# sandyz1000/deep-insight-face

Measured on AMD Instinct MI355X. Metric: faces/sec embedding+match (112x112, 512-d), higher is better.
Workload: dtype f32; 1 GPU; configs[3]: IResNet-100 embed, batch=512/GPU (4096 on 8 GPUs), 1M gallery row-sharded; arch=iresnet100, head=v2, batch_per_gpu=512, global_batch=512, gallery_rows=1000000, gallery_rows_per_gpu=1000000, emd=512, metric=cosine, parallelism=dp1 + gallery row-shard

## Files before the change

deep-insight-face_amd/csrc/conv.hip:

```cpp
#include "gemm_core.hpp"
#include <string>
#include "dif_internal.hpp"
#include "ops.hpp"

#include <stdlib.h>

#include <atomic>
#include <mutex>
#include <set>
#include <type_traits>
#include <utility>

namespace dif {

template <int N>
__device__ __forceinline__ void wait_vmcnt() {
  static_assert(N >= 0 && N < 64, "vmcnt is a 6-bit counter");
  asm volatile("s_waitcnt vmcnt(%0)" ::"n"(N) : "memory");
}


template <int N, int RP, bool PRE, int KMODE = 0>
struct ConvALoader {
  __amdgpu_buffer_rsrc_t rsrc;
// ... 1915 lines not shown
    g_last_kernel = names.insert(std::string("conv_skp_kernel<64x64,") + am_form(AMP + 10) + ",S=" + std::to_string(S) + ">+reduce").first->c_str();
  }
  return 0;
}

template <class T>
static int launch_conv(const ConvArgs& a, hipStream_t st) {
  if constexpr (T::BM == 64 && T::BN == 64) {
    if (const int nw = mt_plan(a)) return launch_conv_mt(a, nw, st);
    if (const int S = sk2_plan(a)) {
      const int emax = (!(a.off & CONV_OFF_BD) && a.w_frag && !(a.dbg & 16384)) ? patch_applies(a) : 0;
      if (emax == PATCH_EMAX_S) return launch_conv_skp<3>(a, S, st);
      if (emax == PATCH_EMAX_L) return launch_conv_skp<5>(a, S, st);
      const bool pw1 = a.KH == 1 && a.KW == 1 && a.pad_t == 0 && a.pad_l == 0 && a.Cin % BK == 0;
      if (pw1) return a.pre_scale ? launch_conv_sk<true, 1>(a, S, st) : launch_conv_sk<false, 1>(a, S, st);
      return a.pre_scale ? launch_conv_sk<true, 0>(a, S, st) : launch_conv_sk<false, 0>(a, S, st);
    }
  }
  constexpr bool kDefaultTile = (T::BM == 64 && T::BN == 64);
  const bool pw = a.KH == 1 && a.KW == 1 && a.pad_t == 0 && a.pad_l == 0 && a.Cin % BK == 0;
  if constexpr (kDefaultTile) {
    const int64_t tiles = ((a.M + T::BM - 1) / T::BM) * (int64_t)((a.Cout + T::BN - 1) / T::BN);
    int64_t slots = 4 * (int64_t)num_cus();
    if (slots > a.sk_max_blocks) slots = a.sk_max_blocks;
    const bool bd = !(a.off & CONV_OFF_BD) && a.w_frag != nullptr;
    if (patch2d_applies(a)) {
      if (t2_applies(a)) return launch_conv_t2(a, st);
      if (bd && conv_bdp_ok(a)) return launch_conv_bdp<T, 6>(a, st);
      return bd ? launch_conv_pre<T, false, 16>(a, st) : launch_conv_pre<T, false, 6>(a, st);
    }
    if (bd && !pw) {
      int emax_tn = patch_applies(a);
      if (emax_tn == 0 && patch_shape(a) && patch_entry_bound(a, 64) <= PATCH_EMAX_X && !(a.dbg & 8192)) emax_tn = PATCH_EMAX_X;
      if (tn_applies(a, emax_tn) && (conv_bdp_ok(a) || (a.dbg & 512)))
        return emax_tn == PATCH_EMAX_X ? launch_conv_tn<PATCH_EMAX_X>(a, st)
                                       : (emax_tn == PATCH_EMAX_L ? launch_conv_tn<PATCH_EMAX_L>(a, st) : launch_conv_tn<PATCH_EMAX_S>(a, st));
    }
    if (bd && !pw && conv_bdp_ok(a)) {
      const int emax = patch_applies(a);
      if (emax == PATCH_EMAX_S) return launch_conv_bdp<T, 3>(a, st);
      if (emax == PATCH_EMAX_L) return launch_conv_bdp<T, 5>(a, st);
    }
    if (a.Cin % 4 == 0 && pipe_applies(a, tiles, a.Kpad / BK, slots)) {
      if (pw && a.pre_scale) return launch_conv_pipe<T, true, 1, 4>(a, st);
      if (pw) return launch_conv_pipe<T, false, 1, 4>(a, st);
      if (!a.pre_scale) return launch_conv_pipe<T, false, 0, 1>(a, st);
    }
  }
  if (pw && a.pre_scale) return launch_conv_pre<T, true, 1>(a, st);
  if (pw) return launch_conv_pre<T, false, 1>(a, st);
  if constexpr (kDefaultTile) {
    {
      const bool bd2 = !(a.off & CONV_OFF_BD) && a.w_frag != nullptr;
      const int emax = patch_applies(a);
      if (bd2 && conv_bdp_ok(a)) {
        if (emax == PATCH_EMAX_S) return launch_conv_bdp<T, 3>(a, st);
        if (emax == PATCH_EMAX_L) return launch_conv_bdp<T, 5>(a, st);
        if (patch2d_applies(a)) return launch_conv_bdp<T, 6>(a, st);
      }
      if (emax == PATCH_EMAX_S) return bd2 ? launch_conv_pre<T, false, 13>(a, st) : launch_conv_pre<T, false, 3>(a, st);
      if (emax == PATCH_EMAX_L) return bd2 ? launch_conv_pre<T, false, 15>(a, st) : launch_conv_pre<T, false, 5>(a, st);
      if (patch2d_applies(a)) return bd2 ? launch_conv_pre<T, false, 16>(a, st) : launch_conv_pre<T, false, 6>(a, st);
    }
  }
  if (a.pre_scale) return launch_conv_pre<T, true, 0>(a, st);
  return launch_conv_pre<T, false, 0>(a, st);
}

template <class T, bool PRE, int AM, int BF3, int LEAN>
static int launch_conv_pre_impl(const ConvArgs& a, hipStream_t st);

template <class T, bool PRE, int AM, int BF3>
static int launch_conv_pre(const ConvArgs& a, hipStream_t st) {
  const bool lean = !(a.dbg & 1024) && a.y_H == a.Ho && a.y_W == a.Wo && a.y_oy == 0 && a.y_ox == 0 && a.y_ld == a.Cout &&
                    a.y_coff == 0 && !a.y_sub && a.Cout % 4 == 0 &&
                    (!a.res || (a.res_stride == 1 && a.res_H == a.Ho && a.res_W == a.Wo)) && (int64_t)a.M * a.Cout * 4 < 0xFFFFFFF0LL;
  if constexpr (BF3) return a.y_sub ? launch_conv_pre_impl<T, PRE, AM, BF3, 2>(a, st) : launch_conv_pre_impl<T, PRE, AM, BF3, 1>(a, st);
  else return lean ? launch_conv_pre_impl<T, PRE, AM, BF3, 1>(a, st) : launch_conv_pre_impl<T, PRE, AM, BF3, 0>(a, st);
}

template <class T, bool PRE, int AM, int BF3, int LEAN>
static int launch_conv_pre_impl(const ConvArgs& a, hipStream_t st) {
  void (*kern)(const ConvArgs) = conv_igemm_kernel<T, PRE, AM, BF3, LEAN>;
  if constexpr (BF3 != 0) {
    if (a.bf_terms == 2) kern = conv_igemm_bf2_kernel<T, PRE, AM, BF3, LEAN>;
  }
  constexpr int AMP = AM % 10;
  constexpr int emax = AMP == 3 ? PATCH_EMAX_S : (AMP == 5 ? PATCH_EMAX_L : 100);
  constexpr int epi_bytes = T::BM * (T::BN + 4) * 4;
  constexpr int bd_bytes = emax * 128 > epi_bytes ? emax * 128 : epi_bytes;
  constexpr int b3p_bytes = bf3p_lds_b(T::BM) > epi_bytes ? bf3p_lds_b(T::BM) : epi_bytes;
  constexpr int lds_bytes = BF3 ? b3p_bytes
                                : (AM >= 10 ? bd_bytes : ((AMP == 3 || AMP == 5 || AMP == 6) ? patch_lds_bytes(emax) : T::LDS_BYTES));
  if (allow_dynamic_lds(reinterpret_cast<const void*>(kern), lds_bytes)) return -1;
  const int64_t tiles = ((a.M + T::BM - 1) / T::BM) * (int64_t)((a.Cout + T::BN - 1) / T::BN);
  const int KS = (BF3 && AM >= 10) ? a.Kpad / (BK * 9) : a.Kpad / BK;
  const int64_t I = tiles * KS;
  if (I >= 0x7fffffffLL) return set_error("conv: iteration space too large");
  int64_t slots = (BF3 ? 512 / T::NT : T::BLOCKS_PER_CU) * (int64_t)num_cus();
  if (slots > a.sk_max_blocks) slots = a.sk_max_blocks;
  int64_t P;
  if (tiles >= 8 * slots || a.Kpad / BK < SK_MIN_KS || (((BF3 && a.bf_terms == 2) || (a.dbg & 2048)) && tiles >= slots) || (a.dbg & 4096)) {
    P = tiles;
  } else {
    P = slots;
    if (P > (I + 3) / 4) P = (I + 3) / 4;
  }
  if (P < 1) P = 1;
  ConvArgs b = a;
  b.fd_howo = make_fastdiv(a.Ho * a.Wo);
  b.fd_wo = make_fastdiv(a.Wo);
  b.fd_cin = make_fastdiv(a.Cin);
  b.fd_kw = make_fastdiv(a.KW);
  b.fd_ks = make_fastdiv(KS);
  b.fd_taps = make_fastdiv(a.KH * a.KW);
  b.fd_wp = make_fastdiv(a.W + 2);
  b.fd_rpi = make_fastdiv(a.H + 1);
  b.fd_t2_w = make_fastdiv(a.W / 8 > 0 ? a.W / 8 : 1);
  b.fd_t2_img = make_fastdiv((a.H / 8) * (a.W / 8) > 0 ? (a.H / 8) * (a.W / 8) : 1);
  if (a.k_order == 1 && a.Cin % BK != 0) return set_error("conv: channel-block-major K order needs Cin %% 32 == 0");
  b.fd_tiles_n = make_fastdiv((a.Cout + T::BN - 1) / T::BN);
  b.epi_fast = LEAN != 0;
  hipLaunchKernelGGL(kern, dim3((unsigned)P), dim3(T::NT), lds_bytes, st, b);
  DIF_HIP(hipGetLastError());
  static const std::string label = kernel_label<T>(BF3 ? "conv_igemm_kernel[split-bf16]" : "conv_igemm_kernel", AM, PRE ? ",preact" : "");
  g_last_kernel = label.c_str();
  return 0;
}

#include "conv_winograd.hpp"

int conv_run(const ConvArgs& a, hipStream_t st) {
  if (a.M <= 0) return 0;
  if (a.Cin % 4 != 0) return set_error("conv: Cin must be a multiple of 4 (got %d)", a.Cin);
  if (a.Cout % 4 != 0) {
    if (a.res) return set_error("conv: a shortcut needs Cout %% 4 == 0 (got %d)", a.Cout);
  } else if (a.y_ld % 4 != 0 || a.y_coff % 4 != 0) {
    return set_error("conv: output view must be 16-byte aligned");
  }
  if (a.y_ld < a.y_coff + a.Cout || a.y_H < a.Ho + a.y_oy || a.y_W < a.Wo + a.y_ox)
    return set_error("conv: output view does not fit its parent tensor");
  if (a.y_sub && (a.Cout % 4 != 0 || a.y_ld != a.Cout || a.y_H != a.Ho || a.y_W != a.Wo))
    return set_error("conv: a subsampled first output needs a plain output geometry");
  if (a.Kpad % BK != 0) return set_error("conv: Kpad must be a multiple of %d", BK);
  if (a.H >= 0x3f00 || a.W >= 0x3f00) return set_error("conv: spatial size too large");
  if ((a.pre_scale == nullptr) != (a.pre_shift == nullptr)) return set_error("conv: pre_scale and pre_shift go together");
  if (!a.sk_slab || !a.sk_flag || a.sk_max_blocks < 1) return set_error("conv: stream-K workspace missing");
  {
    const int64_t howo = (int64_t)a.Ho * a.Wo;
    const int64_t span = (256 + howo - 1) / howo + 1;
    if (span * a.H * a.W * a.Cin * 4 >= 0x7fffffffLL)
      return set_error("conv: a 256-pixel tile spans more than 2 GiB of input (%dx%dx%d)", a.H, a.W, a.Cin);
  }
  if (const int wk = wino_applies(a)) return wk == 2 ? launch_conv_winow(a, st) : launch_conv_wino(a, st);
  const int form = bf3p_applies(a) * 2 + (a.Cout <= 64 ? 1 : 0);
  if (form == 2 && (a.bf_terms == 2 || (a.dbg & 128))) return launch_conv_pre<Tile<4, 1, 1, 4>, false, 13, 1>(a, st);
  switch (form) {
    case 2: return launch_conv_pre<Tile<2, 2, 2, 2>, false, 13, 1>(a, st);
    case 3: return launch_conv_pre<Tile<2, 1, 2, 2>, false, 13, 1>(a, st);
    case 4: return launch_conv_pre<Tile<2, 2, 2, 2>, false, 16, 1>(a, st);
    case 5: return launch_conv_pre<Tile<2, 1, 2, 2>, false, 16, 1>(a, st);
    default: break;
  }
  if (a.Cout <= 32 && !(a.dbg & 8388608)) return launch_conv<Tile<1, 1, 4, 1>>(a, st);
  return launch_conv<Tile<1, 1>>(a, st);
}

}
```

deep-insight-face_amd/csrc/conv_winograd.hpp:

```cpp
namespace wino {
constexpr int BN = 64;
constexpr int KC = 16;
constexpr int64_t MIN_TILES = 64 * 49;
constexpr int WIDE_MAX_HW = 112;
constexpr int64_t WIDE_MIN_IMAGES = 128;
}

template <int TT_, int CPW_, int MIN_BLOCKS_, bool EARLY_REQ_>
struct WinoW {
  static constexpr int TT = TT_;
  static constexpr int CPW = CPW_;
  static constexpr int MIN_BLOCKS = MIN_BLOCKS_;
  static constexpr bool EARLY_REQ = EARLY_REQ_;
  static constexpr int MF = TT / 32;
  static constexpr int NT = 16 / CPW * 64;
  static constexpr int STAGE = 16 * TT * wino::KC;
  static constexpr int LDS_BYTES = 2 * STAGE * 4;
  static_assert(NT / 8 == TT && CPW % 2 == 0, "one loader thread per (tile, channel pair)");
};

__device__ __forceinline__ void wino_bt4(float x0, float x1, float x2, float x3, float& o0, float& o1, float& o2, float& o3) {
  o0 = x0 - x2;
  o1 = x1 + x2;
  o2 = x2 - x1;
  o3 = x1 - x3;
}

__device__ __forceinline__ void wino_input_transform(const float (&d)[16], float (&v)[16]) {
  float t[16];
#pragma unroll
  for (int c = 0; c < 4; ++c) wino_bt4(d[c], d[4 + c], d[8 + c], d[12 + c], t[c], t[4 + c], t[8 + c], t[12 + c]);
#pragma unroll
  for (int r = 0; r < 4; ++r) wino_bt4(t[4 * r], t[4 * r + 1], t[4 * r + 2], t[4 * r + 3], v[4 * r], v[4 * r + 1], v[4 * r + 2], v[4 * r + 3]);
}

template <bool TRACE>
__device__ __forceinline__ unsigned long long wino_stamp() {
  if constexpr (TRACE) return __builtin_amdgcn_s_memrealtime();
  return 0ull;
}
__device__ __forceinline__ void wino_trace_write(const ConvArgs& a, unsigned long long c0, const unsigned long long (&ts)[5]) {
  unsigned long long* t = a.trace + (size_t)blockIdx.x * 8;
  t[0] = ts[2] - ts[1];
  t[1] = ts[1] - ts[0];
  t[2] = ts[3] - ts[2];
  t[3] = ts[4] - ts[3];
  t[4] = (unsigned long long)__builtin_amdgcn_s_getreg((31 << 11) | 4) | ((unsigned long long)__builtin_amdgcn_s_getreg((31 << 11) | 20) << 32);
  t[5] = ts[0];
  t[6] = ts[4];
  t[7] = 3 | ((__builtin_amdgcn_s_memtime() - c0) << 8);
}

template <class S, bool TRACE>
__global__ __launch_bounds__(S::NT, S::MIN_BLOCKS) void conv_wino_kernel(const ConvArgs a, int blocks_m, int nblocks) {
  constexpr int TT = S::TT, CPW = S::CPW, MF = S::MF, KC = wino::KC;
  extern __shared__ __attribute__((aligned(16))) float wino_smem[];
  const int b = xcd_remap((int)blockIdx.x, nblocks);
  const int nt = b / blocks_m, mt = b - nt * blocks_m;
  const int tid = threadIdx.x, lane = tid & 63, wave = tid >> 6;
  const int tw = a.W >> 1, tpi = (a.H >> 1) * tw, ntiles = a.N * tpi;
  const int KS = a.Cin / KC;
  unsigned long long ts[5];
  ts[0] = wino_stamp<TRACE>();
  const unsigned long long tr_c0 = TRACE ? __builtin_amdgcn_s_memtime() : 0ull;

  const int ltile = tid >> 3, cp = tid & 7;
  const int g = mt * TT + ltile;
  const bool tile_ok = g < ntiles;
  int pix0 = 0;
  unsigned vmask = 0;
  if (tile_ok) {
    const int img = g / tpi, rem = g - img * tpi, ty = rem / tw, tx = rem - ty * tw;
    pix0 = (img * a.H + 2 * ty) * a.W + 2 * tx;
#pragma unroll
    for (int p = 0; p < 16; ++p) {
      const int iy = 2 * ty - 1 + (p >> 2), ix = 2 * tx - 1 + (p & 3);
      if (iy >= 0 && iy < a.H && ix >= 0 && ix < a.W) vmask |= 1u << p;
    }
  }
  const int row_b = a.W * a.Cin * 4, pix_b = a.Cin * 4;
  const int lbase = (pix0 - a.W - 1) * pix_b + cp * 8;
  const __amdgpu_buffer_rsrc_t xrs = make_rsrc(a.x, (uint32_t)a.N * (uint32_t)(a.H * a.W) * (uint32_t)pix_b);
  auto dload = [&](int ks, f32x2 (&d)[16]) {
#pragma unroll
    for (int p = 0; p < 16; ++p) {
      const uint32_t off = ((vmask >> p) & 1u) ? (uint32_t)(lbase + (p >> 2) * row_b + (p & 3) * pix_b + ks * (KC * 4)) : OOB;
      d[p] = __builtin_bit_cast(f32x2, __builtin_amdgcn_raw_buffer_load_b64(xrs, off, 0, 0));
    }
  };
  const int vdst = ltile * KC + (((cp >> 1) ^ ((ltile >> 2) & 3)) << 2) + (cp & 1) * 2;
  auto vstore = [&](float* buf, const f32x2 (&d)[16]) {
    float d0[16], d1[16], v0[16], v1[16];
#pragma unroll
    for (int p = 0; p < 16; ++p) {
      d0[p] = d[p][0];
      d1[p] = d[p][1];
    }
    wino_input_transform(d0, v0);
    wino_input_transform(d1, v1);
#pragma unroll
    for (int c = 0; c < 16; ++c) *reinterpret_cast<f32x2*>(buf + c * (TT * KC) + vdst) = f32x2{v0[c], v1[c]};
  };

  const int h = lane >> 5, r32 = lane & 31, sw = (r32 >> 2) & 3;
  const int tiles_n = a.Cout / wino::BN;
  const __amdgpu_buffer_rsrc_t wrs = make_rsrc(a.w_wino, a.w_wino_bytes);
  const uint32_t boff0 = (uint32_t)((CPW * wave * tiles_n + nt) * KS) * 4096u + (uint32_t)lane * 16u;
  const uint32_t bstep = (uint32_t)(tiles_n * KS) * 4096u;
  f32x4 bw[2][2][2];
  auto bload = [&](int j, int ks) {
#pragma unroll
    for (int nf = 0; nf < 2; ++nf)
#pragma unroll
      for (int q = 0; q < 2; ++q)
        bw[j & 1][nf][q] = buf_load4(wrs, boff0 + (uint32_t)j * bstep + (uint32_t)ks * 4096u + (uint32_t)(nf * 2 + q) * 1024u);
  };
  int aoff[2];
#pragma unroll
  for (int q = 0; q < 2; ++q) aoff[q] = r32 * KC + (((2 * h + q) ^ sw) << 2);
  f32x4 av[2][MF][2];
  auto aread = [&](const float* buf, int j) {
#pragma unroll
    for (int mf = 0; mf < MF; ++mf)
#pragma unroll
      for (int q = 0; q < 2; ++q)
        av[j & 1][mf][q] = *reinterpret_cast<const f32x4*>(buf + (CPW * wave + j) * (TT * KC) + mf * 32 * KC + aoff[q]);
  };
  f32x16 acc[CPW][MF][2];
#pragma unroll
  for (int j = 0; j < CPW; ++j)
#pragma unroll
    for (int mf = 0; mf < MF; ++mf)
#pragma unroll
      for (int nf = 0; nf < 2; ++nf)
#pragma unroll
        for (int r = 0; r < 16; ++r) acc[j][mf][nf][r] = 0.f;
  auto mfma = [&](int j) {
#pragma unroll
    for (int q = 0; q < 2; ++q)
#pragma unroll
      for (int t = 0; t < 4; ++t)
#pragma unroll
        for (int mf = 0; mf < MF; ++mf)
#pragma unroll
          for (int nf = 0; nf < 2; ++nf)
            acc[j][mf][nf] = __builtin_amdgcn_mfma_f32_32x32x2f32(av[j & 1][mf][q][t], bw[j & 1][nf][q][t], acc[j][mf][nf], 0, 0, 0);
  };

  {
    f32x2 d[16];
    dload(0, d);
    bload(0, 0);
    bload(1, 0);
    vstore(wino_smem, d);
    lds_barrier();
    ts[1] = wino_stamp<TRACE>();
    for (int ks = 0; ks < KS; ++ks) {
      const float* cur = wino_smem + (ks & 1) * S::STAGE;
      float* nxt = wino_smem + ((ks + 1) & 1) * S::STAGE;
      const bool more = ks + 1 < KS;
      if (more) dload(ks + 1, d);
      aread(cur, 0);
      aread(cur, 1);
#pragma unroll
      for (int j = 0; j < CPW; ++j) {
        mfma(j);
        if (j + 2 < CPW) {
          aread(cur, j + 2);
          bload(j + 2, ks);
        } else if (more) {
          bload(j + 2 - CPW, ks + 1);
        }
      }
      if (more) vstore(nxt, d);
      lds_barrier();
    }
  }
  ts[2] = wino_stamp<TRACE>();

  const int c4 = cp * 4;
  const uint32_t bytes = (uint32_t)a.M * (uint32_t)a.Cout * 4u;
  const __amdgpu_buffer_rsrc_t y_rsrc = make_rsrc(a.y, a.y ? bytes : 0u);
  const __amdgpu_buffer_rsrc_t y2_rsrc = make_rsrc(a.y2, a.y2 ? bytes : 0u);
  const __amdgpu_buffer_rsrc_t res_rsrc = make_rsrc(a.res, a.res ? bytes : 0u);
  const bool has_res = a.res != nullptr;
  const int act = a.act, act2 = a.act2;
#pragma unroll
  for (int nf = 0; nf < 2; ++nf) {
    const int c = nt * wino::BN + nf * 32 + c4;
    f32x4 sc, sh, al, sc2, sh2, al2, rv[4];
    uint32_t voff[4];
    if constexpr (S::EARLY_REQ) {
      sc = load4_or(a.scale, c, 1.f), sh = load4_or(a.shift, c, 0.f), al = load4_or(a.alpha, c, 0.f);
      sc2 = load4_or(a.scale2, c, 1.f), sh2 = load4_or(a.shift2, c, 0.f), al2 = load4_or(a.alpha2, c, 0.f);
#pragma unroll
      for (int p = 0; p < 4; ++p) {
        const int pix = pix0 + (p >> 1) * a.W + (p & 1);
        voff[p] = tile_ok ? ((uint32_t)pix * (uint32_t)a.Cout + (uint32_t)c) * 4u : OOB;
        rv[p] = has_res ? buf_load4(res_rsrc, voff[p]) : f32x4{0.f, 0.f, 0.f, 0.f};
      }
      __builtin_amdgcn_sched_barrier(0);
    }
#pragma unroll
    for (int j = 0; j < CPW; ++j)
#pragma unroll
      for (int mf = 0; mf < MF; ++mf)
#pragma unroll
        for (int r = 0; r < 16; ++r)
          wino_smem[(CPW * wave + j) * (TT * 32) + (mf * 32 + frag_row(lane, r)) * 32 + r32] = acc[j][mf][nf][r];
    lds_barrier();
    f32x4 m[16];
#pragma unroll
    for (int k = 0; k < 16; ++k) m[k] = *reinterpret_cast<const f32x4*>(wino_smem + k * (TT * 32) + ltile * 32 + c4);
    f32x4 yv[4];
    {
      f32x4 s0[4], s1[4];
#pragma unroll
      for (int jj = 0; jj < 4; ++jj) {
        s0[jj] = m[jj] + m[4 + jj] + m[8 + jj];
        s1[jj] = m[4 + jj] - m[8 + jj] - m[12 + jj];
      }
      yv[0] = s0[0] + s0[1] + s0[2];
      yv[1] = s0[1] - s0[2] - s0[3];
      yv[2] = s1[0] + s1[1] + s1[2];
      yv[3] = s1[1] - s1[2] - s1[3];
    }
    if constexpr (!S::EARLY_REQ) {
      sc = load4_or(a.scale, c, 1.f), sh = load4_or(a.shift, c, 0.f), al = load4_or(a.alpha, c, 0.f);
      sc2 = load4_or(a.scale2, c, 1.f), sh2 = load4_or(a.shift2, c, 0.f), al2 = load4_or(a.alpha2, c, 0.f);
#pragma unroll
      for (int p = 0; p < 4; ++p) {
        const int pix = pix0 + (p >> 1) * a.W + (p & 1);
        voff[p] = tile_ok ? ((uint32_t)pix * (uint32_t)a.Cout + (uint32_t)c) * 4u : OOB;
        rv[p] = has_res ? buf_load4(res_rsrc, voff[p]) : f32x4{0.f, 0.f, 0.f, 0.f};
      }
    }
#pragma unroll
    for (int p = 0; p < 4; ++p) {
      f32x4 v, v2;
      epilogue4(yv[p], sc, sh, al, act, has_res, rv[p], sc2, sh2, al2, act2, v, v2);
      __builtin_amdgcn_raw_buffer_store_b128(__builtin_bit_cast(u32x4, v), y_rsrc, voff[p], 0, 0);
      __builtin_amdgcn_raw_buffer_store_b128(__builtin_bit_cast(u32x4, v2), y2_rsrc, voff[p], 0, 0);
    }
    lds_barrier();
    ts[3 + nf] = wino_stamp<TRACE>();
  }
  if constexpr (TRACE)
    if (tid == 0) wino_trace_write(a, tr_c0, ts);
}

static int wino_applies(const ConvArgs& a) {
  if (!a.w_wino || a.wino_level < 1 || a.KH != 3 || a.KW != 3 || a.stride != 1 || a.pad_t != 1 || a.pad_l != 1) return 0;
  if (a.Ho != a.H || a.Wo != a.W || (a.H & 1) || (a.W & 1)) return 0;
  const bool wide = a.H > 16 || a.W > 16;
  if (wide && (a.wino_level < 2 || a.H > wino::WIDE_MAX_HW || a.W > wino::WIDE_MAX_HW)) return 0;
  if (a.Cin % 32 != 0 || a.Cout % wino::BN != 0 || a.pre_scale || a.y_sub) return 0;
  if (!(a.y_H == a.Ho && a.y_W == a.Wo && a.y_oy == 0 && a.y_ox == 0 && a.y_ld == a.Cout && a.y_coff == 0)) return 0;
  if (a.res && (a.res_stride != 1 || a.res_H != a.Ho || a.res_W != a.Wo)) return 0;
  if ((int64_t)a.M * a.Cout * 4 >= 0x7fffffffLL || (int64_t)a.M * a.Cin * 4 >= 0x7fffffffLL) return 0;
  if ((int64_t)16 * a.Cin * a.Cout * 4 > (int64_t)a.w_wino_bytes) return 0;
  const int64_t tpi = (int64_t)(a.H / 2) * (a.W / 2);
  if (wide) return a.N * tpi >= wino::WIDE_MIN_IMAGES * tpi ? 2 : 0;
  return a.N * tpi >= wino::MIN_TILES ? 1 : 0;
}

template <class S>
static int launch_wino(const ConvArgs& a, hipStream_t st, const char* name) {
  const auto kern = a.trace ? conv_wino_kernel<S, true> : conv_wino_kernel<S, false>;
  if (allow_dynamic_lds(reinterpret_cast<const void*>(kern), S::LDS_BYTES)) return -1;
  const int64_t ntiles = (int64_t)a.N * (a.H / 2) * (a.W / 2);
  const int blocks_m = (int)((ntiles + S::TT - 1) / S::TT), tiles_n = a.Cout / wino::BN;
  const int64_t nblocks = (int64_t)blocks_m * tiles_n;
  if (nblocks >= 0x7fffffffLL) return set_error("conv: too many tiles");
  hipLaunchKernelGGL(kern, dim3((unsigned)nblocks), dim3(S::NT), S::LDS_BYTES, st, a, blocks_m, (int)nblocks);
  DIF_HIP(hipGetLastError());
  g_last_kernel = name;
  return 0;
}

static int launch_conv_wino(const ConvArgs& a, hipStream_t st) {
  if (a.wino_level >= 2 && !(a.dbg & 16777216)) return launch_wino<WinoW<32, 4, 2, true>>(a, st, "conv_wino_kernel<F(2x2,3x3),32 tiles x 64>");
  return launch_wino<WinoW<64, 2, 1, false>>(a, st, "conv_wino_kernel<F(2x2,3x3),64 tiles x 64>");
}

static int launch_conv_winow(const ConvArgs& a, hipStream_t st) {
  if (a.dbg & 65536) return launch_wino<WinoW<64, 2, 2, true>>(a, st, "conv_winow_kernel<F(2x2,3x3),64 tiles x 64>");
  return launch_wino<WinoW<32, 4, 2, true>>(a, st, "conv_winow_kernel<F(2x2,3x3),32 tiles x 64>");
}
```

deep-insight-face_amd/csrc/net.hip:

```cpp
#include "net.hpp"

#include <math.h>
#include <stdio.h>
#include <stdlib.h>
#include <string.h>

#include <algorithm>
#include <map>

#include "../../include/dif.h"
#include "dif_internal.hpp"
#include "gemm_core.hpp"

namespace dif {

static const float EPS_RESNET = 1.001e-5f;
static const float EPS_KERAS = 1e-3f;
static const float EPS_IRESNET = 1e-5f;

Net::~Net() { release_device(); }

void Net::release_device() {
  for (Lane& L : lanes) {
    if (L.stream) (void)hipStreamDestroy(L.stream);
// ... 832 lines not shown
    for (const char* const* t = option_names(); *t; ++t) known |= !strcmp(*t, key);
    if (!known) return set_error("dif_net_set_option: unknown option '%s'", key);
  }
  auto flag = [&](unsigned bit) {
    conv_off = value ? (conv_off & ~bit) : (conv_off | bit);
    return 0;
  };
  const bool pre = !finalized;
  if (!strcmp(key, "pipe")) return use_pipe = value != 0, 0;
  if (!strcmp(key, "bdp")) {
    if (value < 0 || value > 2) return set_error("dif_net_set_option: 'bdp' takes 0, 1 or 2");
    return use_bdp = value, 0;
  }
  if (!strcmp(key, "stem")) return use_stem = value != 0, 0;
  if (!strcmp(key, "dbg")) return conv_dbg = value, 0;
  if (!strcmp(key, "wino")) {
    if (value < 0 || value > 2) return set_error("dif_net_set_option: 'wino' takes 0, 1 or 2");
    return use_wino = value, 0;
  }
  if (!strcmp(key, "patch")) return flag(CONV_OFF_PATCH);
  if (!strcmp(key, "patch2d")) return flag(CONV_OFF_PATCH2D);
  if (!strcmp(key, "bd")) return flag(CONV_OFF_BD);
  if (!strcmp(key, "t2")) return flag(CONV_OFF_T2);
  if (!strcmp(key, "tn")) return flag(CONV_OFF_TN);
  if (!strcmp(key, "sk2")) return flag(CONV_OFF_SK2);
  if (!strcmp(key, "mt")) return flag(CONV_OFF_MT);
  if (!strcmp(key, "bf16x3")) {
    if (!pre && compute_bf16x3 != (value != 0))
      return set_error("dif_net_set_option: 'bf16x3' must be chosen before dif_net_finalize");
    return compute_bf16x3 = value != 0, 0;
  }
  if (!strcmp(key, "bf_terms")) {
    if (value != 2 && value != 3) return set_error("dif_net_set_option: 'bf_terms' takes 2 or 3");
    return bf_terms = value, 0;
  }
  if (!strcmp(key, "lane_prio")) {
    if (!pre) return set_error("dif_net_set_option: 'lane_prio' must be chosen before dif_net_finalize");
    return opt_lane_prio = value, 0;
  }
  if (!strcmp(key, "ysub") || !strcmp(key, "lane_split")) {
    if (!pre) return set_error("dif_net_set_option: '%s' must be chosen before dif_net_finalize", key);
    if (key[0] == 'y') use_ysub = value != 0;
    else opt_lane_split = value < 0 ? -1 : (value != 0);
    return 0;
  }
  return set_error("dif_net_set_option: option '%s' is listed but not handled", key);
}

int Net::finalize(int mb) {
  if (mb <= 0) return set_error("max_batch must be positive");
  if (const char* env = getenv("DIF_OPTIONS")) {
    std::string all(env);
    size_t pos = 0;
    while (pos < all.size()) {
      size_t end = all.find(',', pos);
      if (end == std::string::npos) end = all.size();
      const std::string kv = all.substr(pos, end - pos);
      const size_t eq = kv.find('=');
      if (eq == std::string::npos || eq == 0) return set_error("DIF_OPTIONS: expected key=value, got '%s'", kv.c_str());
      if (set_option(kv.substr(0, eq).c_str(), atoi(kv.c_str() + eq + 1))) return -1;
      pos = end + 1;
    }
  }
  for (const Param& p : params)
    if (!p.set) return set_error("parameter '%s' was never set", p.name.c_str());
  release_device();
  max_batch = mb;

  for (Op& op : ops) {
    std::vector<float> scale, shift;
    if (op.kind == OP_CONV) {
      const int taps = op.KH * op.KW;
      const int K = taps * op.Cin;
      op.Kpad = (K + BK - 1) / BK * BK;
      op.k_order = (taps > 1 && op.Cin % BK == 0 && op.Cin_true == op.Cin) ? 1 : 0;
      std::vector<float> packed((size_t)op.Cout * op.Kpad, 0.f);
      const float* w = params[op.w].data.data();
      for (int t = 0; t < taps; ++t)
        for (int ci = 0; ci < op.Cin_true; ++ci) {
          const int64_t src_row = op.chw_flatten ? ((int64_t)ci * taps + t) : ((int64_t)t * op.Cin_true + ci);
          const float* src = w + src_row * op.Cout;
          const size_t kk = op.k_order == 1 ? ((size_t)(ci / BK) * taps + t) * BK + ci % BK : (size_t)t * op.Cin + ci;
          for (int co = 0; co < op.Cout; ++co) packed[(size_t)co * op.Kpad + kk] = src[co];
        }
      if (upload(this, packed, &op.d_w)) return -1;
      op.d_w_raw = nullptr;
      op.stem_mfma = false;
      const bool stem_shape = use_stem && op.Cin_true == 3 && op.Cin == 4 && op.res < 0 && !op.pre_bn.valid() &&
                              !op.chw_flatten && tensors[op.y >= 0 ? op.y : op.y2].parent < 0;
      if (stem_shape && op.KH == 3 && op.KW == 3 && op.stride == 1 && op.pad_t == 1 && op.pad_l == 1 && op.Cout == 32) {
        if (upload(this, params[op.w].data, &op.d_w_raw)) return -1;
      } else if (stem_shape && stem_mfma_applies(op.KH, op.KW, op.stride, op.pad_t, op.pad_l, op.Cout)) {
        if (upload(this, params[op.w].data, &op.d_w_raw)) return -1;
        op.stem_mfma = true;
      }
      op.d_w3f = nullptr;
      op.w3f_bytes = 0;
      if (compute_bf16x3 && op.k_order == 1 && op.KH == 3 && op.KW == 3 && op.stride == 1 && op.pad_t == 1 && op.pad_l == 1 &&
          !op.pre_bn.valid() && conv_bf3p_form(tensors[op.x].H, tensors[op.x].W, true, op.Cout) != 0) {
        const int KS = op.Kpad / BK, NT32 = (op.Cout + 31) / 32;
        std::vector<uint16_t> wf((size_t)NT32 * KS * 3072, 0);
        size_t o = 0;
        for (int nt = 0; nt < NT32; ++nt)
          for (int ks = 0; ks < KS; ++ks)
            for (int s2 = 0; s2 < 2; ++s2) {
              uint16_t* blk = wf.data() + o;
              o += 3 * 512;
              for (int ln = 0; ln < 64; ++ln)
                for (int t = 0; t < 8; ++t) {
                  const int row = nt * 32 + (ln & 31);
                  float r = row < op.Cout ? packed[(size_t)row * op.Kpad + (size_t)ks * BK + 16 * s2 + 8 * (ln >> 5) + t] : 0.f;
                  for (int p3 = 0; p3 < 3; ++p3) {
                    const uint16_t b = f32_to_bf16_rne(r);
                    blk[p3 * 512 + ln * 8 + t] = b;
                    r -= bf16_to_f32(b);
                  }
                }
            }
        if ((uint64_t)wf.size() * 2 < 0xFFFFFFF0ull) {
          void* d = nullptr;
          DIF_HIP(hipMalloc(&d, wf.size() * sizeof(uint16_t)));
          allocs.push_back(d);
          DIF_HIP(hipMemcpy(d, wf.data(), wf.size() * sizeof(uint16_t), hipMemcpyHostToDevice));
          op.d_w3f = d;
          op.w3f_bytes = (uint32_t)(wf.size() * sizeof(uint16_t));
        }
      }
      op.d_w_frag = nullptr;
      op.w_frag_bytes = 0;
      if (!op.d_w3f && op.k_order == 1 && op.KH == 3 && op.KW == 3 && op.stride == 1 && op.pad_t == 1 && op.pad_l == 1 &&
          !op.pre_bn.valid()) {
        const int KS = op.Kpad / BK, NT32 = (op.Cout + 31) / 32;
        std::vector<float> frag((size_t)NT32 * 32 * op.Kpad, 0.f);
        size_t o = 0;
        for (int nt = 0; nt < NT32; ++nt)
          for (int ks = 0; ks < KS; ++ks)
            for (int s2 = 0; s2 < 2; ++s2)
              for (int u = 0; u < 2; ++u)
                for (int hh = 0; hh < 2; ++hh)
                  for (int nn = 0; nn < 32; ++nn)
                    for (int t = 0; t < 4; ++t, ++o) {
                      const int row = nt * 32 + nn;
                      if (row < op.Cout) frag[o] = packed[(size_t)row * op.Kpad + (size_t)ks * BK + 16 * s2 + 8 * hh + 4 * u + t];
                    }
        if ((uint64_t)frag.size() * 4 < 0xFFFFFFF0ull) {
          if (upload(this, frag, &op.d_w_frag)) return -1;
          op.w_frag_bytes = (uint32_t)(frag.size() * 4);
        }
      }
      op.d_w_wino = nullptr;
      op.w_wino_bytes = 0;
      {
        const TensorDesc& xd = tensors[op.x];
        const TensorDesc& yd = tensors[op.y >= 0 ? op.y : op.y2];
        if (use_wino && !compute_bf16x3 && op.KH == 3 && op.KW == 3 && op.stride == 1 && op.pad_t == 1 && op.pad_l == 1 &&
            !op.pre_bn.valid() && !op.chw_flatten && !op.y_sub && op.Cin_true == op.Cin && op.Cin % BK == 0 &&
            op.Cout % 64 == 0 && xd.H % 2 == 0 && xd.W % 2 == 0 && yd.H == xd.H && yd.W == xd.W &&
            ((xd.H <= 16 && xd.W <= 16) || (use_wino >= 2 && xd.H <= 112 && xd.W <= 112)) &&
            (uint64_t)16 * op.Cin * op.Cout * 4 < 0xFFFFFFF0ull) {
          static const double G[4][3] = {{1, 0, 0}, {0.5, 0.5, 0.5}, {0.5, -0.5, 0.5}, {0, 0, 1}};
          const int KS16 = op.Cin / 16, NTn = op.Cout / 64;
          std::vector<float> u((size_t)16 * op.Cin * op.Cout);
          const float* w = params[op.w].data.data();
          for (int ci = 0; ci < op.Cin; ++ci)
            for (int co = 0; co < op.Cout; ++co) {
              double gk[3][3], tg[4][3];
              for (int t = 0; t < 9; ++t) gk[t / 3][t % 3] = w[((size_t)t * op.Cin + ci) * op.Cout + co];
              for (int i = 0; i < 4; ++i)
                for (int k = 0; k < 3; ++k) tg[i][k] = G[i][0] * gk[0][k] + G[i][1] * gk[1][k] + G[i][2] * gk[2][k];
              const int ks = ci / 16, rem = ci % 16, ln = (rem / 8) * 32 + co % 32, q = (rem % 8) / 4, t4 = rem % 4;
              const int nt = co / 64, nf = (co % 64) / 32;
              for (int i = 0; i < 4; ++i)
                for (int j = 0; j < 4; ++j) {
                  const double v = tg[i][0] * G[j][0] + tg[i][1] * G[j][1] + tg[i][2] * G[j][2];
                  const size_t c = (size_t)(4 * i + j);
                  u[(((((c * NTn + nt) * KS16 + ks) * 2 + nf) * 2 + q) * 64 + ln) * 4 + t4] = (float)v;
                }
            }
          if (upload(this, u, &op.d_w_wino)) return -1;
          op.w_wino_bytes = (uint32_t)(u.size() * 4);
        }
      }
      op.d_w_f16 = nullptr;
      op.w_f16_bytes = 0;
      {
        const bool pw1 = op.KH == 1 && op.KW == 1 && op.pad_t == 0 && op.pad_l == 0 && op.Cin % BK == 0;
        if ((pw1 || (op.k_order == 1 && op.Cin % BK == 0)) && !op.d_w_raw) {
          const int nch = op.Kpad / 16, NT16 = (op.Cout + 15) / 16;
          std::vector<float> f16((size_t)NT16 * nch * 256, 0.f);
          size_t o = 0;
          for (int ct = 0; ct < NT16; ++ct)
            for (int c = 0; c < nch; ++c)
              for (int ln = 0; ln < 64; ++ln)
                for (int t = 0; t < 4; ++t, ++o) {
                  const int row = ct * 16 + (ln & 15);
                  if (row < op.Cout) f16[o] = packed[(size_t)row * op.Kpad + (size_t)c * 16 + 4 * (ln >> 4) + t];
                }
          if ((uint64_t)f16.size() * 4 < 0xFFFFFFF0ull) {
            if (upload(this, f16, &op.d_w_f16)) return -1;
            op.w_f16_bytes = (uint32_t)(f16.size() * 4);
          }
        }
      }
      fold(this, op.bn, op.bias, op.Cout, &scale, &shift);
      if (!scale.empty() && upload(this, scale, &op.d_scale)) return -1;
      if (!shift.empty() && upload(this, shift, &op.d_shift)) return -1;
      if (op.alpha >= 0 && upload(this, params[op.alpha].data, &op.d_alpha)) return -1;
      if (op.alpha < 0 && op.const_alpha != 0.f &&
          upload(this, std::vector<float>((size_t)op.Cout, op.const_alpha), &op.d_alpha))
        return -1;
    } else if (op.kind == OP_GDCTAIL) {
      if (upload(this, params[op.w].data, &op.d_w)) return -1;
      if (upload(this, params[op.w_pw].data, &op.d_w_pw)) return -1;
      if (upload(this, params[op.w_dense].data, &op.d_w_dense)) return -1;
      fold(this, op.bn, -1, op.Cin, &scale, &shift);
      if (!scale.empty() && upload(this, scale, &op.d_scale)) return -1;
      if (!shift.empty() && upload(this, shift, &op.d_shift)) return -1;
    } else if (op.kind == OP_DWFULL || op.kind == OP_DWCONV) {
      if (upload(this, params[op.w].data, &op.d_w)) return -1;
      fold(this, op.bn, -1, op.Cout, &scale, &shift);
      if (!scale.empty() && upload(this, scale, &op.d_scale)) return -1;
      if (!shift.empty() && upload(this, shift, &op.d_shift)) return -1;
    }
    if (op.pre_bn.valid()) {
      fold(this, op.pre_bn, -1, op.Cin, &scale, &shift);
      if (upload(this, scale, &op.d_pre_scale)) return -1;
      if (upload(this, shift, &op.d_pre_shift)) return -1;
    }
    if (op.y2 >= 0) {
      fold(this, op.bn2, -1, op.Cout, &scale, &shift);
      if (!scale.empty() && upload(this, scale, &op.d_scale2)) return -1;
      if (!shift.empty() && upload(this, shift, &op.d_shift2)) return -1;
      if (op.alpha2 >= 0 && upload(this, params[op.alpha2].data, &op.d_alpha2)) return -1;
    }
  }

  for (Op& P : ops) {
    if (!use_ysub || P.kind != OP_CONV || P.y < 0 || P.y2 < 0 || P.y_sub || is_output(P.y) || tensors[P.y].parent >= 0 ||
        tensors[P.y2].parent >= 0 || P.Cout % 4 != 0)
      continue;
    bool viewed = false;
    for (const TensorDesc& t : tensors) viewed |= t.parent == P.y;
    Op* reader = nullptr;
    int readers = 0;
    for (Op& D : ops) {
      if (&D == &P) continue;
      const int uses = (D.x == P.y) + (D.res == P.y) + (D.y == P.y) + (D.y2 == P.y);
      if (uses) {
        readers += uses;
        reader = &D;
      }
    }
    if (viewed || readers != 1 || reader->kind != OP_CONV || reader->x != P.y) continue;
    if (reader->KH != 1 || reader->KW != 1 || reader->stride != 2 || reader->pad_t != 0 || reader->pad_l != 0) continue;
    TensorDesc& t = tensors[P.y];
    P.y_sub = true;
    t.H = (t.H + 1) / 2;
    t.W = (t.W + 1) / 2;
    reader->stride = 1;
  }

  for (TensorDesc& t : tensors) t.first_def = t.last_use = t.buf = -1;
  auto R = [&](int t) { return t < 0 ? t : root_of(t); };
  for (int i = 0; i < (int)ops.size(); ++i) {
    const Op& op = ops[i];
    for (int t : {R(op.y), R(op.y2)})
      if (t >= 0 && tensors[t].first_def < 0) tensors[t].first_def = i;
    for (int t : {R(op.x), R(op.res), R(op.y), R(op.y2)})
      if (t >= 0) tensors[t].last_use = std::max(tensors[t].last_use, i);
  }
  tensors[output_tensor].last_use = (int)ops.size();
  for (int e : extra_outputs) tensors[e].last_use = (int)ops.size();
  buf_elems.clear();
  std::vector<int> free_list;
  for (int i = 0; i < (int)ops.size(); ++i) {
    const Op& op = ops[i];
    for (int t : {R(op.y), R(op.y2)}) {
      if (t < 0 || is_output(t) || tensors[t].buf >= 0) continue;
      const int64_t need = tensors[t].elems();
      int best = -1;
      for (int k = 0; k < (int)free_list.size(); ++k) {
        const int b = free_list[k];
        if (buf_elems[b] >= need && (best < 0 || buf_elems[b] < buf_elems[free_list[best]])) best = k;
      }
      if (best >= 0) {
        tensors[t].buf = free_list[best];
        free_list.erase(free_list.begin() + best);
      } else {
        buf_elems.push_back(need);
        tensors[t].buf = (int)buf_elems.size() - 1;
      }
    }
    for (int t : {R(op.x), R(op.res), R(op.y), R(op.y2)})
      if (t >= 0 && !is_output(t) && tensors[t].last_use == i && tensors[t].buf >= 0) {
        if (std::find(free_list.begin(), free_list.end(), tensors[t].buf) == free_list.end())
          free_list.push_back(tensors[t].buf);
      }
  }
  sk_max_blocks = conv_max_blocks();
  if (const char* e = getenv("DIF_SK_SPIN_LIMIT")) sk_spin_limit = atoi(e);
  int n_conv = 0;
  for (const Op& op : ops) n_conv += op.kind == OP_CONV;
  const double per_launch = flops_per_image() * (max_batch / 2) / (n_conv > 0 ? n_conv : 1);
  const bool long_launches = per_launch >= 10e9;
  int nl = getenv("DIF_STREAMS") ? atoi(getenv("DIF_STREAMS")) : 2;
  lane_split = (opt_lane_split >= 0 ? opt_lane_split : (long_launches ? 0 : 1)) != 0;
  if (nl < 1) nl = 1;
  if (nl > 8) nl = 8;
  if (max_batch < lane_min_images()) nl = 1;
  lanes.assign(nl, Lane());
  DIF_HIP(hipEventCreateWithFlags(&ev_start, hipEventDisableTiming));
// ... 507 lines not shown
```

Measured before the change: 8286 faces/s.

## Extend Winograd 3x3 conv to odd-sized maps and subsampled-output convs

Widens Winograd F(2x2,3x3) coverage to two shapes that previously fell back to the implicit-GEMM path. The first is odd spatial maps up to 16x16 (e.g. 7x7 in IResNet), handled by padding tiles and masking out-of-range outputs via the input validity mask. The second is convs whose first output is stride-2 subsampled (y_sub), handled by storing only the top-left pixel of each 2x2 tile. This cuts the multiply count for those layers, at the cost of wasted work on padded tiles for odd maps and a new kernel variant to validate.

After: 8560 faces/s, median of 6. 1.03x the previous value.

```diff
diff --git a/deep-insight-face_amd/csrc/conv.hip b/deep-insight-face_amd/csrc/conv.hip
--- a/deep-insight-face_amd/csrc/conv.hip
+++ b/deep-insight-face_amd/csrc/conv.hip
@@ -2091,7 +2091,8 @@
     if (span * a.H * a.W * a.Cin * 4 >= 0x7fffffffLL)
       return set_error("conv: a 256-pixel tile spans more than 2 GiB of input (%dx%dx%d)", a.H, a.W, a.Cin);
   }
-  if (const int wk = wino_applies(a)) return wk == 2 ? launch_conv_winow(a, st) : launch_conv_wino(a, st);
+  if (const int wk = wino_applies(a); wk && !(wk == 3 && (a.dbg & 33554432)))
+    return wk == 3 ? launch_conv_winox(a, st) : wk == 2 ? launch_conv_winow(a, st) : launch_conv_wino(a, st);
   const int form = bf3p_applies(a) * 2 + (a.Cout <= 64 ? 1 : 0);
   if (form == 2 && (a.bf_terms == 2 || (a.dbg & 128))) return launch_conv_pre<Tile<4, 1, 1, 4>, false, 13, 1>(a, st);
   switch (form) {
diff --git a/deep-insight-face_amd/csrc/conv_winograd.hpp b/deep-insight-face_amd/csrc/conv_winograd.hpp
--- a/deep-insight-face_amd/csrc/conv_winograd.hpp
+++ b/deep-insight-face_amd/csrc/conv_winograd.hpp
@@ -4,6 +4,8 @@
 constexpr int64_t MIN_TILES = 64 * 49;
 constexpr int WIDE_MAX_HW = 112;
 constexpr int64_t WIDE_MIN_IMAGES = 128;
+constexpr int ODD_MAX_HW = 16;
+constexpr int64_t ODD_MIN_TILES = 128 * 16;
 }
 
 template <int TT_, int CPW_, int MIN_BLOCKS_, bool EARLY_REQ_>
@@ -12,11 +14,20 @@
   static constexpr int CPW = CPW_;
   static constexpr int MIN_BLOCKS = MIN_BLOCKS_;
   static constexpr bool EARLY_REQ = EARLY_REQ_;
+  static constexpr bool ODD = false;
+  static constexpr bool YSUB = false;
   static constexpr int MF = TT / 32;
   static constexpr int NT = 16 / CPW * 64;
   static constexpr int STAGE = 16 * TT * wino::KC;
   static constexpr int LDS_BYTES = 2 * STAGE * 4;
   static_assert(NT / 8 == TT && CPW % 2 == 0, "one loader thread per (tile, channel pair)");
+};
+
+template <bool ODD_, bool YSUB_>
+struct WinoX : WinoW<32, 4, 2, true> {
+  static constexpr bool ODD = ODD_;
+  static constexpr bool YSUB = YSUB_;
+  static_assert(!(ODD_ && YSUB_), "y_sub is admitted on even maps only");
 };
 
 __device__ __forceinline__ void wino_bt4(float x0, float x1, float x2, float x3, float& o0, float& o1, float& o2, float& o3) {
@@ -57,8 +68,9 @@
   extern __shared__ __attribute__((aligned(16))) float wino_smem[];
   const int b = xcd_remap((int)blockIdx.x, nblocks);
   const int nt = b / blocks_m, mt = b - nt * blocks_m;
-  const int tid = threadIdx.x, lane = tid & 63, wave = tid >> 6;
-  const int tw = a.W >> 1, tpi = (a.H >> 1) * tw, ntiles = a.N * tpi;
+  const int tid = threadIdx.x, lane = tid & 63;
+  const int wave = (S::ODD || S::YSUB) ? __builtin_amdgcn_readfirstlane(tid >> 6) : tid >> 6;
+  const int tw = S::ODD ? (a.W + 1) >> 1 : a.W >> 1, tpi = (S::ODD ? (a.H + 1) >> 1 : a.H >> 1) * tw, ntiles = a.N * tpi;
   const int KS = a.Cin / KC;
   unsigned long long ts[5];
   ts[0] = wino_stamp<TRACE>();
@@ -180,7 +192,7 @@
 
   const int c4 = cp * 4;
   const uint32_t bytes = (uint32_t)a.M * (uint32_t)a.Cout * 4u;
-  const __amdgpu_buffer_rsrc_t y_rsrc = make_rsrc(a.y, a.y ? bytes : 0u);
+  const __amdgpu_buffer_rsrc_t y_rsrc = make_rsrc(a.y, a.y ? (S::YSUB ? (uint32_t)ntiles * (uint32_t)a.Cout * 4u : bytes) : 0u);
   const __amdgpu_buffer_rsrc_t y2_rsrc = make_rsrc(a.y2, a.y2 ? bytes : 0u);
   const __amdgpu_buffer_rsrc_t res_rsrc = make_rsrc(a.res, a.res ? bytes : 0u);
   const bool has_res = a.res != nullptr;
@@ -196,7 +208,10 @@
 #pragma unroll
       for (int p = 0; p < 4; ++p) {
         const int pix = pix0 + (p >> 1) * a.W + (p & 1);
-        voff[p] = tile_ok ? ((uint32_t)pix * (uint32_t)a.Cout + (uint32_t)c) * 4u : OOB;
+        if constexpr (S::ODD)
+          voff[p] = ((vmask >> (5 + 4 * (p >> 1) + (p & 1))) & 1u) ? ((uint32_t)pix * (uint32_t)a.Cout + (uint32_t)c) * 4u : OOB;
+        else
+          voff[p] = tile_ok ? ((uint32_t)pix * (uint32_t)a.Cout + (uint32_t)c) * 4u : OOB;
         rv[p] = has_res ? buf_load4(res_rsrc, voff[p]) : f32x4{0.f, 0.f, 0.f, 0.f};
       }
       __builtin_amdgcn_sched_barrier(0);
@@ -231,7 +246,10 @@
 #pragma unroll
       for (int p = 0; p < 4; ++p) {
         const int pix = pix0 + (p >> 1) * a.W + (p & 1);
-        voff[p] = tile_ok ? ((uint32_t)pix * (uint32_t)a.Cout + (uint32_t)c) * 4u : OOB;
+        if constexpr (S::ODD)
+          voff[p] = ((vmask >> (5 + 4 * (p >> 1) + (p & 1))) & 1u) ? ((uint32_t)pix * (uint32_t)a.Cout + (uint32_t)c) * 4u : OOB;
+        else
+          voff[p] = tile_ok ? ((uint32_t)pix * (uint32_t)a.Cout + (uint32_t)c) * 4u : OOB;
         rv[p] = has_res ? buf_load4(res_rsrc, voff[p]) : f32x4{0.f, 0.f, 0.f, 0.f};
       }
     }
@@ -239,7 +257,11 @@
     for (int p = 0; p < 4; ++p) {
       f32x4 v, v2;
       epilogue4(yv[p], sc, sh, al, act, has_res, rv[p], sc2, sh2, al2, act2, v, v2);
-      __builtin_amdgcn_raw_buffer_store_b128(__builtin_bit_cast(u32x4, v), y_rsrc, voff[p], 0, 0);
+      if constexpr (S::YSUB) {
+        if (p == 0) __builtin_amdgcn_raw_buffer_store_b128(__builtin_bit_cast(u32x4, v), y_rsrc, tile_ok ? ((uint32_t)g * (uint32_t)a.Cout + (uint32_t)c) * 4u : OOB, 0, 0);
+      } else {
+        __builtin_amdgcn_raw_buffer_store_b128(__builtin_bit_cast(u32x4, v), y_rsrc, voff[p], 0, 0);
+      }
       __builtin_amdgcn_raw_buffer_store_b128(__builtin_bit_cast(u32x4, v2), y2_rsrc, voff[p], 0, 0);
     }
     lds_barrier();
@@ -251,15 +273,18 @@
 
 static int wino_applies(const ConvArgs& a) {
   if (!a.w_wino || a.wino_level < 1 || a.KH != 3 || a.KW != 3 || a.stride != 1 || a.pad_t != 1 || a.pad_l != 1) return 0;
-  if (a.Ho != a.H || a.Wo != a.W || (a.H & 1) || (a.W & 1)) return 0;
+  if (a.Ho != a.H || a.Wo != a.W) return 0;
+  const bool odd = (a.H & 1) || (a.W & 1), rest = odd || a.y_sub;
   const bool wide = a.H > 16 || a.W > 16;
+  if (rest && (a.wino_level < 2 || (odd && (a.y_sub || a.H > wino::ODD_MAX_HW || a.W > wino::ODD_MAX_HW || a.H < 3 || a.W < 3)))) return 0;
   if (wide && (a.wino_level < 2 || a.H > wino::WIDE_MAX_HW || a.W > wino::WIDE_MAX_HW)) return 0;
-  if (a.Cin % 32 != 0 || a.Cout % wino::BN != 0 || a.pre_scale || a.y_sub) return 0;
+  if (a.Cin % 32 != 0 || a.Cout % wino::BN != 0 || a.pre_scale) return 0;
   if (!(a.y_H == a.Ho && a.y_W == a.Wo && a.y_oy == 0 && a.y_ox == 0 && a.y_ld == a.Cout && a.y_coff == 0)) return 0;
   if (a.res && (a.res_stride != 1 || a.res_H != a.Ho || a.res_W != a.Wo)) return 0;
   if ((int64_t)a.M * a.Cout * 4 >= 0x7fffffffLL || (int64_t)a.M * a.Cin * 4 >= 0x7fffffffLL) return 0;
   if ((int64_t)16 * a.Cin * a.Cout * 4 > (int64_t)a.w_wino_bytes) return 0;
-  const int64_t tpi = (int64_t)(a.H / 2) * (a.W / 2);
+  const int64_t tpi = (int64_t)((a.H + 1) / 2) * ((a.W + 1) / 2);
+  if (rest) return a.N >= wino::WIDE_MIN_IMAGES && (!odd || a.N * tpi >= wino::ODD_MIN_TILES) ? 3 : 0;
   if (wide) return a.N * tpi >= wino::WIDE_MIN_IMAGES * tpi ? 2 : 0;
   return a.N * tpi >= wino::MIN_TILES ? 1 : 0;
 }
@@ -268,7 +293,7 @@
 static int launch_wino(const ConvArgs& a, hipStream_t st, const char* name) {
   const auto kern = a.trace ? conv_wino_kernel<S, true> : conv_wino_kernel<S, false>;
   if (allow_dynamic_lds(reinterpret_cast<const void*>(kern), S::LDS_BYTES)) return -1;
-  const int64_t ntiles = (int64_t)a.N * (a.H / 2) * (a.W / 2);
+  const int64_t ntiles = S::ODD ? (int64_t)a.N * ((a.H + 1) / 2) * ((a.W + 1) / 2) : (int64_t)a.N * (a.H / 2) * (a.W / 2);
   const int blocks_m = (int)((ntiles + S::TT - 1) / S::TT), tiles_n = a.Cout / wino::BN;
   const int64_t nblocks = (int64_t)blocks_m * tiles_n;
   if (nblocks >= 0x7fffffffLL) return set_error("conv: too many tiles");
@@ -287,3 +312,8 @@
   if (a.dbg & 65536) return launch_wino<WinoW<64, 2, 2, true>>(a, st, "conv_winow_kernel<F(2x2,3x3),64 tiles x 64>");
   return launch_wino<WinoW<32, 4, 2, true>>(a, st, "conv_winow_kernel<F(2x2,3x3),32 tiles x 64>");
 }
+
+static int launch_conv_winox(const ConvArgs& a, hipStream_t st) {
+  if (a.y_sub) return launch_wino<WinoX<false, true>>(a, st, "conv_winox_kernel<F(2x2,3x3),32 tiles x 64,ysub>");
+  return launch_wino<WinoX<true, false>>(a, st, "conv_winox_kernel<F(2x2,3x3),32 tiles x 64,odd>");
+}
diff --git a/deep-insight-face_amd/csrc/net.hip b/deep-insight-face_amd/csrc/net.hip
--- a/deep-insight-face_amd/csrc/net.hip
+++ b/deep-insight-face_amd/csrc/net.hip
@@ -1008,11 +1008,12 @@
       op.w_wino_bytes = 0;
       {
         const TensorDesc& xd = tensors[op.x];
-        const TensorDesc& yd = tensors[op.y >= 0 ? op.y : op.y2];
+        const TensorDesc& yd = tensors[op.y >= 0 && !op.y_sub ? op.y : op.y2];
+        const bool odd = xd.H % 2 != 0 || xd.W % 2 != 0, rest = odd || op.y_sub;
         if (use_wino && !compute_bf16x3 && op.KH == 3 && op.KW == 3 && op.stride == 1 && op.pad_t == 1 && op.pad_l == 1 &&
-            !op.pre_bn.valid() && !op.chw_flatten && !op.y_sub && op.Cin_true == op.Cin && op.Cin % BK == 0 &&
-            op.Cout % 64 == 0 && xd.H % 2 == 0 && xd.W % 2 == 0 && yd.H == xd.H && yd.W == xd.W &&
-            ((xd.H <= 16 && xd.W <= 16) || (use_wino >= 2 && xd.H <= 112 && xd.W <= 112)) &&
+            !op.pre_bn.valid() && !op.chw_flatten && !(rest && use_wino < 2) && !(odd && op.y_sub) && op.Cin_true == op.Cin && op.Cin % BK == 0 &&
+            op.Cout % 64 == 0 && yd.H == xd.H && yd.W == xd.W &&
+            ((xd.H <= 16 && xd.W <= 16) || (use_wino >= 2 && !odd && xd.H <= 112 && xd.W <= 112)) &&
             (uint64_t)16 * op.Cin * op.Cout * 4 < 0xFFFFFFF0ull) {
           static const double G[4][3] = {{1, 0, 0}, {0.5, 0.5, 0.5}, {0.5, -0.5, 0.5}, {0, 0, 1}};
           const int KS16 = op.Cin / 16, NTn = op.Cout / 64;
```
